# cxjyxxme/deep-online-video-stabilization

Measured on AMD Instinct MI355X. Metric: stabilized frames/sec (720p, before_ch=31), higher is better.
Workload: dtype f32 (bf16x3 split MFMA, f32 accumulate); 1 GPU; BASELINE.json configs[1]: v2_93 net, 1280x720, 1 stream(s)/GPU, batch=1 per stream, 13-ch stack from a 32-deep ring (lags 1,2,4,8,16,32; --before-ch 31 ignored as in the reference), ResNet-v2-50 regressor + 4x4 multi-grid warp + feedback; one independent stream set per GPU (replicas only); height=720, width=1280, streams_per_gpu=1, refine=1, operand_mode=4, launches_per_frame=64, hip_graph=True

## Files before the change

deep-online-video-stabilization_amd/csrc/conv.h:

```cpp
#pragma once
#include "common.h"

struct ConvArgs {
    const float* x;
    const float* w;
    float* y;
    const float* bias;
    const float* in_scale;
    const float* in_shift;
    const float* residual;
    const float* out_scale;
    const float* out_shift;
    const float* out_floor;
    float* partial;
    int N, H, W, Cin, Ho, Wo, Cout, KH, KW, stride, pad;
    int up;
    int res_H, res_W, res_stride;
    int relu_out;
    int x_ld, res_ld;
    int M, K;
    int splitk, steps_per_split;
    int cin_real;
    unsigned div_hw_mul, div_hw_shift, div_w_mul, div_w_shift;
    int rowrun;
    int in_scale_expected;
    int xcd_swizzle;
};

size_t conv_plan(ConvArgs& a);
struct Prof;
int conv_launch(const ConvArgs& a, hipStream_t st, Prof* prof = nullptr, int bf16_operands = 0, const float* w_img = nullptr,
                bool lowk_ring = false);

enum ConvFamily {
    CONV_IGEMM,
    CONV_RING,
    CONV_RING_KG,
    CONV_RING_PRO,
    CONV_PACKED,
    CONV_PACKED_KG2
};
struct ConvRoute {
    int family;
    int tile, bk, nbuf;
    int mode;
    int operand;
    int kg, pro;
    int reduce;
    int prof_kind;
};
ConvRoute conv_route(const ConvArgs& a, int operand_mode, bool has_image, bool bound, bool lowk_ring = false );
const char* conv_prof_kind_name(int kind);
size_t conv_weight_image_floats(int Cout, int K);
int launch_weight_split_image(const float* w, int Cout, int K, float* img, hipStream_t st);
struct WeightImageTable { long w_off[64], img_off[64], tprefix[65]; int Cout[64], K[64]; int n; };
void weight_image_table_add(WeightImageTable& t, long w_off, long img_off, int Cout, int K);
int launch_weight_split_images(const float* w_base, float* img_base, const WeightImageTable& t, hipStream_t st);
int conv_reduce_launches(const ConvArgs& a, int operand_mode = 0);

struct ConvPair { int m_tower, x_tower_floats ; long dx, dy, dres, dscale; };
bool conv_pair_supported(const ConvArgs& a);
int conv_launch_pair(const ConvArgs& a, const ConvPair& pr, hipStream_t st, Prof* prof = nullptr,
                     const float* w_img = nullptr );

bool conv_b2b_supported(const ConvArgs& c2, const ConvArgs& c3);
int conv_b2b_launch(const ConvArgs& c2, const ConvArgs& c3, hipStream_t st, Prof* prof = nullptr);

static inline void sn_fastdiv_make(unsigned d, unsigned& mul, unsigned& shift) {
    unsigned l = 0;
    while ((1ull << l) < d) ++l;
    mul = (unsigned)((((1ull << l) - d) << 32) / d + 1);
    shift = l;
}
#ifdef __HIPCC__
__device__ __forceinline__ int sn_fastdiv(int n, unsigned mul, unsigned shift) {
    return (int)((__umulhi(mul, (unsigned)n) + (unsigned)n) >> shift);
}
#endif
```

deep-online-video-stabilization_amd/csrc/conv.hip:

```cpp
#include "conv.h"
#include "prof.h"
#include <climits>
#include <cstdio>
#include <cstdlib>
#include <algorithm>
#include <string>
#include <vector>

#include "conv_kernel.h"
#include "conv_ring_kernel.h"
#include "conv_b2b_kernel.h"

template <int PAIR>
__device__ __forceinline__ void conv_splitk_reduce_body(const ConvArgs& p, const ConvPair& pr) {
    const size_t q = (size_t)blockIdx.x * 256 + threadIdx.x;
    const int c4n = p.Cout / 4;
    if (q >= (size_t)p.M * c4n) return;
    const int m = (int)(q / c4n);
    const int n = (int)(q - (size_t)m * c4n) * 4;
    const bool t1 = PAIR && m >= pr.m_tower;
    const size_t slab = (size_t)p.M * p.Cout;
    const float* src = p.partial + (size_t)m * p.Cout + n;
    float4 s = *reinterpret_cast<const float4*>(src);
    for (int z = 1; z < p.splitk; ++z) {
        const float4 t = *reinterpret_cast<const float4*>(src + z * slab);
        s.x += t.x; s.y += t.y; s.z += t.z; s.w += t.w;
    }
    if (p.bias != nullptr) {
        const float4 b = *reinterpret_cast<const float4*>(p.bias + n);
        s.x += b.x; s.y += b.y; s.z += b.z; s.w += b.w;
    }
    if (p.residual != nullptr) {
        size_t ri;
        if (p.res_stride == 1 && p.res_H == p.Ho && p.res_W == p.Wo) {
            ri = (size_t)m * p.res_ld + n;
        } else {
            const int img = sn_fastdiv(m, p.div_hw_mul, p.div_hw_shift);
            const int rr = m - img * (p.Ho * p.Wo);
            const int oy = sn_fastdiv(rr, p.div_w_mul, p.div_w_shift), ox = rr - oy * p.Wo;
            ri = (((size_t)img * p.res_H + oy * p.res_stride) * p.res_W + ox * p.res_stride) * p.res_ld + n;
        }
        const float4 t = *reinterpret_cast<const float4*>(p.residual + (t1 ? pr.dres : 0) + ri);
        s.x += t.x; s.y += t.y; s.z += t.z; s.w += t.w;
    }
    if (p.out_scale != nullptr) {
        const float4 a = *reinterpret_cast<const float4*>(p.out_scale + n), b = *reinterpret_cast<const float4*>(p.out_shift + n);
        s.x = __builtin_fmaf(s.x, a.x, b.x); s.y = __builtin_fmaf(s.y, a.y, b.y);
        s.z = __builtin_fmaf(s.z, a.z, b.z); s.w = __builtin_fmaf(s.w, a.w, b.w);
    }
    if (p.out_scale != nullptr && p.out_floor != nullptr) {
        const float4 f = *reinterpret_cast<const float4*>(p.out_floor + n);
        s.x = fmaxf(s.x, f.x); s.y = fmaxf(s.y, f.y); s.z = fmaxf(s.z, f.z); s.w = fmaxf(s.w, f.w);
    } else if (p.relu_out) {
        s.x = fmaxf(s.x, 0.f); s.y = fmaxf(s.y, 0.f); s.z = fmaxf(s.z, 0.f); s.w = fmaxf(s.w, 0.f);
    }
    *reinterpret_cast<float4*>(p.y + (t1 ? pr.dy : 0) + (size_t)m * p.Cout + n) = s;
}
__global__ __launch_bounds__(256) void conv_splitk_reduce_kernel(const ConvArgs p) {
    conv_splitk_reduce_body<0>(p, ConvPair{});
}
__global__ __launch_bounds__(256) void conv_splitk_reduce_pair_kernel(const ConvArgs p, const ConvPair pr) {
    conv_splitk_reduce_body<1>(p, pr);
}

enum TileId { T128x128 = 0, T128x64 = 1, T64x64 = 2 };

static void tile_dims(int t, int& bm, int& bn) {
    bm = (t == T64x64) ? 64 : 128;
    bn = (t == T128x128) ? 128 : 64;
}

static int env_int(const char* name, int dflt) {
    const char* v = getenv(name);
    return v ? atoi(v) : dflt;
}

struct ConvSwitches {
    int tile = env_int("STABNET_CONV_TILE", -1), splitk = env_int("STABNET_CONV_SPLITK", -1);
    int bk16 = env_int("STABNET_CONV_BK16", 0);
    int nbuf = env_int("STABNET_CONV_NBUF", 0);
    int tuning_table = env_int("STABNET_CONV_TUNING_TABLE", 1);
    int split_below = env_int("STABNET_CONV_SPLIT_BELOW", 400), split_target = env_int("STABNET_CONV_SPLIT_TARGET", 448);
    int xcd = env_int("STABNET_CONV_XCD", 1);
    int ring = env_int("STABNET_CONV_RING", 1), ring_wgs_per_cu = env_int("STABNET_CONV_RING_WGS_PER_CU", 3);
    int lowk_igemm = env_int("STABNET_CONV_LOWK_IGEMM", 1);
    int ring_pro = env_int("STABNET_CONV_RING_PRO", 1);
    int kgroups = env_int("STABNET_CONV_KGROUPS", 1), kgroups_pro = env_int("STABNET_CONV_KGROUPS_PRO", 1);
    int packed_kg2 = env_int("STABNET_CONV_PACKED_KG2", 1), packed_kg3 = env_int("STABNET_CONV_PACKED_KG3", 1);
    int packed_pro = env_int("STABNET_CONV_PACKED_PRO", 1);
    int packed_wgs_per_cu = env_int("STABNET_CONV_PACKED_WGS_PER_CU", 2);
    int b2b = env_int("STABNET_CONV_B2B", 1), b2b_wgs_per_cu = env_int("STABNET_CONV_B2B_WGS_PER_CU", 2);
};
static const ConvSwitches& sw() {
    static const ConvSwitches s;
    return s;
}

static int g_force_tile = -2, g_force_split = -1;
static int force_tile() { return g_force_tile == -2 ? sw().tile : g_force_tile; }
static int force_split() { return g_force_tile == -2 ? sw().splitk : g_force_split; }

static int conv_bk(const ConvArgs& a) { return (a.rowrun || (a.Cin % 32 == 0 && !sw().bk16)) ? 32 : 16; }
static int conv_total_steps(const ConvArgs& a) {
    if (a.rowrun) return a.KH * cdiv(a.KW * a.Cin, 32);
    return a.KH * a.KW * (a.Cin / conv_bk(a));
}

struct TuneEntry { int M, Cout, K, KH, ring, splitk; };
#include "conv_tuning_table.h"
#include "conv_tuning_table_packed.h"
static int g_tuning_profile = 0;
static std::vector<TuneEntry> g_tuning_runtime;

static int tuning_lookup(int M, int Cout, int K, int KH, int ring) {
    for (const TuneEntry& e : g_tuning_runtime)
        if (e.M == M && e.Cout == Cout && e.K == K && e.KH == KH && e.ring == ring) return e.splitk;
    if (sw().tuning_table && g_tuning_profile == 1)
        for (const TuneEntry& e : g_tuning_packed)
            if (e.M == M && e.Cout == Cout && e.K == K && e.KH == KH && e.ring == ring) return e.splitk;
    if (sw().tuning_table)
        for (const TuneEntry& e : g_tuning_builtin)
            if (e.M == M && e.Cout == Cout && e.K == K && e.KH == KH && e.ring == ring) return e.splitk;
    return 0;
}

static int pick_tile(const ConvArgs& a, int& splitk) {
    if (force_tile() >= 0) {
        const int steps0 = conv_total_steps(a);
        splitk = force_split() > 0 ? std::min(force_split(), steps0) : 1;
        return force_tile();
    }
    const int total_steps = conv_total_steps(a);
    const long blocks = (long)cdiv(a.M, 64) * cdiv(a.Cout, 64);
    const bool ring_path = a.rowrun || (a.in_scale_expected == 0 && a.up == 1 && a.Cin % 32 == 0);
    int s = tuning_lookup(a.M, a.Cout, a.K, a.KH, ring_path ? 1 : 0);
    const int thr = sw().split_below, target = sw().split_target;
    if (s > 0) {
        s = std::min(s, std::max(1, total_steps / 2));
    } else if (blocks < thr && a.Cout % 4 == 0) {
        s = (int)((target + blocks / 2) / blocks);
        s = std::min(s, std::max(1, total_steps / 8));
        s = std::min(s, 32);
    } else {
// ... 9 lines not shown
    a.K = a.rowrun ? a.KH * 32 * cdiv(a.KW * a.Cin, 32) : a.KH * a.KW * a.Cin;
    if (a.x_ld == 0) a.x_ld = a.Cin;
    if (a.res_ld == 0) a.res_ld = a.Cout;
    sn_fastdiv_make((unsigned)(a.Ho * a.Wo), a.div_hw_mul, a.div_hw_shift);
    sn_fastdiv_make((unsigned)a.Wo, a.div_w_mul, a.div_w_shift);
    int splitk = 1;
    (void)pick_tile(a, splitk);
    const int total_steps = conv_total_steps(a);
    a.steps_per_split = cdiv(total_steps, splitk);
    a.splitk = cdiv(total_steps, a.steps_per_split);
    return a.splitk > 1 ? (size_t)a.splitk * a.M * a.Cout * sizeof(float) : 0;
}

static void igemm_variant(const ConvArgs& a, int bm, int bn, int bk, int mode, int operand, int& nbuf_out, int& bf16_out) {
    const int nbuf = sw().nbuf;
    bf16_out = (bm == 64 && bn == 64 && bk == 32) ? operand : 0;
    const bool one_stage = nbuf == 1 || (nbuf == 0 && mode == 0 && bm == 64 && bn == 64 && a.M >= 32768);
    nbuf_out = (bf16_out != 1 && one_stage) ? 1 : 2;
}

static bool ring_eligible(const ConvArgs& a, int tile, bool has_prologue, bool lowk_ring = false) {
    if (a.rowrun) return true;
    if (!lowk_ring && sw().lowk_igemm && a.KH == 1 && a.KW == 1 && a.Cin == 64 && a.x_ld == a.Cin && a.out_floor == nullptr) return false;
    return sw().ring && tile == T64x64 && !has_prologue && a.up == 1 && a.Cin % 32 == 0 && !sw().bk16;
}

static bool ring_pro_vectors_ok(const ConvArgs& a) {
    if (a.in_scale == nullptr || a.in_shift == nullptr) return true;
    const long d = (long)(a.in_shift - a.in_scale);
    return d >= 0 && d < (1L << 30);
}
static bool ring_pro_geometry(const ConvArgs& a, int operand, bool has_prologue) {
    return sw().ring_pro && sw().ring && operand != 1 && !sw().bk16 && has_prologue && a.KH == 1 && a.KW == 1 && a.stride == 1 && a.pad == 0 &&
           a.up == 1 && a.Cin % 32 == 0 && !a.rowrun && a.x_ld == a.Cin;
}
static bool ring_pro_eligible(const ConvArgs& a, int operand) {
    return ring_pro_geometry(a, operand, a.in_scale != nullptr) && a.out_scale == nullptr && a.out_floor == nullptr && ring_pro_vectors_ok(a);
}

static int conv_kgroups(const ConvArgs& a, int operand, bool ring, bool has_prologue) {
    if (!sw().kgroups || a.splitk < 2 || operand == 1) return 1;
    if (a.steps_per_split * a.splitk != conv_total_steps(a)) return 1;
    if (ring && a.splitk == 3 && !a.rowrun) return 3;
    if (sw().kgroups_pro && !ring && a.splitk == 2 && ring_pro_geometry(a, operand, has_prologue) && ring_pro_vectors_ok(a)) return 2;
    return 1;
}

static int route_prof_kind(const ConvRoute& r) {
    switch (r.family) {
        case CONV_IGEMM:
            return PK_KERNEL_CONV_BASE + r.mode * 6 + r.tile * 2 + (r.bk == 32 ? 1 : 0) + (r.nbuf == 1 ? 18 : 0) + 36 * r.operand;
        case CONV_PACKED: return PK_KERNEL_CONV_PACKED + (r.pro ? 3 : r.mode);
        case CONV_PACKED_KG2: return PK_KERNEL_CONV_PACKED + (r.pro ? 6 : 4 + r.mode);
        default: break;
    }
    const int split = r.operand >= 2 ? PK_KERNEL_CONV_SPLIT + 8 * (r.operand - 2) : 0;
    if (r.family == CONV_RING) return split ? split + r.mode : PK_KERNEL_CONV_RING + r.mode + (r.operand ? 3 : 0);
    if (r.family == CONV_RING_PRO) return split ? split + 5 : PK_KERNEL_CONV_KG + 2;
    if (r.kg == 2) return split ? split + 6 : PK_KERNEL_CONV_KG + 3;
    return split ? split + 3 + r.mode : PK_KERNEL_CONV_KG + r.mode;
}

ConvRoute conv_route(const ConvArgs& a, int operand_mode, bool has_image, bool bound, bool lowk_ring) {
    const ConvSwitches& s = sw();
    const bool image = operand_mode == 4 && has_image;
    const int op = operand_mode == 4 ? 0 : operand_mode;
    int splitk_unused = 1;
    const int t = pick_tile(a, splitk_unused);
    const bool t64 = t == T64x64, bk32 = conv_bk(a) == 32;
    const bool has_pro = bound ? a.in_scale != nullptr : a.in_scale_expected != 0;
    const bool ring = ring_eligible(a, t, has_pro, lowk_ring && image);
    const bool slabs = !bound || a.splitk == 1 || a.partial != nullptr;
    int kg = t64 ? conv_kgroups(a, op, ring, has_pro) : 1;
    if (image && s.packed_kg3 && ring && kg == 3 && a.K % 32 == 0 && slabs) kg = 1;
    const bool pro = kg == 1 && !ring && t64 && bk32 && (bound ? ring_pro_eligible(a, op) : ring_pro_geometry(a, op, has_pro));
    const bool packed_pro = image && s.packed_pro && !ring && t64 && bk32 && ring_pro_geometry(a, op, has_pro) &&
                            (!bound || a.out_floor == nullptr)  && ring_pro_vectors_ok(a) && slabs;
    if (packed_pro) kg = 1;
    const bool packed = (image && ring && kg == 1 && a.K % 32 == 0) || packed_pro;
    const bool packed_kg2 = packed && s.packed_kg2 && a.splitk == 2 && !a.rowrun && a.steps_per_split * 2 == conv_total_steps(a);
    if (packed_kg2) kg = 2;

    ConvRoute r{};
    r.tile = t;
    r.bk = bk32 ? 32 : 16;
    r.mode = (a.up > 1 || a.rowrun) ? 2 : (a.pad == 0 ? 0 : 1);
    r.operand = op;
    r.kg = kg;
    r.reduce = (a.splitk > 1 && kg == 1) ? 1 : 0;
    if (packed) {
        r.family = packed_kg2 ? CONV_PACKED_KG2 : CONV_PACKED;
        r.operand = 4;
        r.pro = packed_pro ? 1 : 0;
    } else if (pro) {
        r.family = CONV_RING_PRO;
        r.pro = 1;
    } else if (kg > 1) {
        r.family = CONV_RING_KG;
        r.pro = kg == 2 ? 1 : 0;
    } else if (ring) {
        r.family = CONV_RING;
    } else {
        int bm, bn;
        tile_dims(t, bm, bn);
        r.family = CONV_IGEMM;
        igemm_variant(a, bm, bn, r.bk, r.mode, op, r.nbuf, r.operand);
    }
    r.prof_kind = route_prof_kind(r);
    return r;
}

int conv_reduce_launches(const ConvArgs& a, int operand_mode) {
    return a.splitk < 2 ? 0 : conv_route(a, operand_mode, operand_mode == 4, false).reduce;
}

const char* conv_prof_kind_name(int kind) {
    static const std::vector<std::string> names = [] {
        std::vector<std::string> v(PK_KERNEL_CONV_BASE + 144);
        char buf[96];
        auto ring = [&](int family, int mode, int operand, int kg, int pro) {
            ConvRoute r{};
            r.family = family; r.mode = mode; r.operand = operand; r.kg = kg; r.pro = pro;
            snprintf(buf, sizeof(buf), "conv_ring_f32_kernel<%d, %d, %d, %d>", mode, operand, kg, pro);
            v[route_prof_kind(r)] = buf;
        };
        for (int operand = 0; operand < 4; ++operand) {
            for (int mode = 0; mode < 3; ++mode) ring(CONV_RING, mode, operand, 1, 0);
            if (operand == 1) continue;
            ring(CONV_RING_KG, 0, operand, 3, 0); ring(CONV_RING_KG, 1, operand, 3, 0);
            ring(CONV_RING_PRO, 0, operand, 1, 1); ring(CONV_RING_KG, 0, operand, 2, 1);
        }
        for (int mode = 0; mode < 3; ++mode) ring(CONV_PACKED, mode, 4, 1, 0);
        ring(CONV_PACKED, 0, 4, 1, 1);
        ring(CONV_PACKED_KG2, 0, 4, 2, 0); ring(CONV_PACKED_KG2, 1, 4, 2, 0); ring(CONV_PACKED_KG2, 0, 4, 2, 1);
        for (int i = 0; i < 144; ++i) {
            ConvRoute r{};
            r.family = CONV_IGEMM;
            r.operand = i / 36; r.nbuf = 2 - i / 18 % 2; r.mode = i / 6 % 3; r.tile = i / 2 % 3; r.bk = (i & 1) ? 32 : 16;
            int bm, bn;
            tile_dims(r.tile, bm, bn);
            snprintf(buf, sizeof(buf), "conv_igemm_f32_kernel<%d, %d, %d, %d, %d, %d, %d, %d>", bm, bn, r.bk, bm / 2, bn / 2, r.mode, r.nbuf, r.operand);
            v[route_prof_kind(r)] = buf;
        }
        for (int i = 0; i < 4; ++i) {
            snprintf(buf, sizeof(buf), "conv_igemm_f32_pair_kernel<64, 64, %d, 32, 32, %d>", (i & 1) ? 32 : 16, i / 2);
            v[PK_KERNEL_CONV_PAIR + i] = buf;
        }
        v[PK_KERNEL_CONV_B2B] = "conv_b2b_f32_kernel<2>";
        v[PK_KERNEL_CONV_B2B + 1] = "conv_b2b_f32_kernel<4>";
        return v;
    }();
    return (kind >= 0 && kind < (int)names.size() && !names[kind].empty()) ? names[kind].c_str() : nullptr;
}

template <int BM, int BN, int BK, int WM, int WN, int MODE, int NBUF, int BF16 = 0>
static int launch_one_nb(const ConvArgs& a, hipStream_t st) {
    constexpr size_t lds_op = NBUF * (size_t)(BM + BN) * (BK + 4) * sizeof(float);
    constexpr size_t lds_epi = 4 * (size_t)SN_EPI_WAVE_BYTES;
    constexpr size_t lds = lds_op > lds_epi ? lds_op : lds_epi;
    static bool configured = false;
    auto kern = conv_igemm_f32_kernel<BM, BN, BK, WM, WN, MODE, NBUF, BF16>;
    if (!configured) {
        if (lds > 64 * 1024) {
            hipError_t e = hipFuncSetAttribute(reinterpret_cast<const void*>(kern),
                                               hipFuncAttributeMaxDynamicSharedMemorySize, (int)lds);
            if (e != hipSuccess) {
                stabnet_set_error("conv: hipFuncSetAttribute(%zu B LDS) failed: %s", lds, hipGetErrorString(e));
                return STABNET_ERR_LAUNCH;
            }
        }
        configured = true;
    }
    dim3 grid(cdiv(a.M, BM), cdiv(a.Cout, BN), a.splitk);
    kern<<<grid, 256, lds, st>>>(a);
    SN_LAUNCH_CHECK("conv_igemm_f32_kernel");
    return STABNET_OK;
}

template <int BM, int BN, int BK, int WM, int WN, int MODE>
static int launch_one_t(const ConvRoute& r, const ConvArgs& a, hipStream_t st) {
    if constexpr (BM == 64 && BN == 64 && BK == 32) {
        if (r.operand == 1) return launch_one_nb<BM, BN, BK, WM, WN, MODE, 2, 1>(a, st);
        else if (r.operand == 2) return r.nbuf == 1 ? launch_one_nb<BM, BN, BK, WM, WN, MODE, 1, 2>(a, st) : launch_one_nb<BM, BN, BK, WM, WN, MODE, 2, 2>(a, st);
        else if (r.operand == 3) return r.nbuf == 1 ? launch_one_nb<BM, BN, BK, WM, WN, MODE, 1, 3>(a, st) : launch_one_nb<BM, BN, BK, WM, WN, MODE, 2, 3>(a, st);
    }
    return r.nbuf == 1 ? launch_one_nb<BM, BN, BK, WM, WN, MODE, 1>(a, st) : launch_one_nb<BM, BN, BK, WM, WN, MODE, 2>(a, st);
}
// ... 20 lines not shown
    static int cached = 0;
    if (cached == 0) {
        int dev = 0, n = 0;
        if (hipGetDevice(&dev) != hipSuccess || hipDeviceGetAttribute(&n, hipDeviceAttributeMultiprocessorCount, dev) != hipSuccess || n <= 0) {
            stabnet_set_error("conv: cannot read the CU count");
            return STABNET_ERR_LAUNCH;
        }
        cached = n;
    }
    cus = cached;
    return STABNET_OK;
}
static int g_reserved_cus = 0;
static int usable_cus(int cus) { return std::max(cus / 8, cus - std::max(0, g_reserved_cus)); }

template <int B>
static bool launch_ring_operand(const ConvRoute& r, const ConvArgs& a, int grid, hipStream_t st) {
    const int key = 100 * r.mode + 10 * r.kg + r.pro;
    if (key == 10) { conv_ring_f32_kernel<0, B><<<grid, 256, 0, st>>>(a); return true; }
    if (key == 110) { conv_ring_f32_kernel<1, B><<<grid, 256, 0, st>>>(a); return true; }
    if (key == 210) { conv_ring_f32_kernel<2, B><<<grid, 256, 0, st>>>(a); return true; }
    if constexpr (B != 1) {
        if (key == 11) { conv_ring_f32_kernel<0, B, 1, 1><<<grid, 256, 0, st>>>(a); return true; }
        if (key == 21) { conv_ring_f32_kernel<0, B, 2, 1><<<grid, 512, 0, st>>>(a); return true; }
    }
    if constexpr (B == 0 || B == 2 || B == 3) {
        if (key == 30) { conv_ring_f32_kernel<0, B, 3><<<grid, 768, 0, st>>>(a); return true; }
        if (key == 130) { conv_ring_f32_kernel<1, B, 3><<<grid, 768, 0, st>>>(a); return true; }
    }
    if constexpr (B == 4) {
        if (key == 20) { conv_ring_f32_kernel<0, B, 2, 0><<<grid, 512, 0, st>>>(a); return true; }
        if (key == 120) { conv_ring_f32_kernel<1, B, 2, 0><<<grid, 512, 0, st>>>(a); return true; }
    }
    return false;
}

static int launch_ring_route(const ConvRoute& r, const ConvArgs& a, hipStream_t st) {
    int cus = 0;
    if (const int rc = device_cus(cus)) return rc;
    const int per_cu = r.kg > 1 ? 1 : (r.operand == 4 ? sw().packed_wgs_per_cu : sw().ring_wgs_per_cu);
    const long ntiles = (long)cdiv(a.M, 64) * cdiv(a.Cout, 64) * (r.kg > 1 ? 1 : a.splitk);
    const int grid = (int)std::min<long>(ntiles, (long)per_cu * usable_cus(cus));
    bool ok = false;
    switch (r.operand) {
        case 0: ok = launch_ring_operand<0>(r, a, grid, st); break;
        case 1: ok = launch_ring_operand<1>(r, a, grid, st); break;
        case 2: ok = launch_ring_operand<2>(r, a, grid, st); break;
        case 3: ok = launch_ring_operand<3>(r, a, grid, st); break;
        case 4: ok = launch_ring_operand<4>(r, a, grid, st); break;
        default: break;
    }
    SN_REQUIRE(ok, "conv: no conv_ring_f32_kernel<%d, %d, %d, %d>", r.mode, r.operand, r.kg, r.pro);
    SN_LAUNCH_CHECK("conv_ring_f32_kernel");
    return STABNET_OK;
}

size_t conv_weight_image_floats(int Cout, int K) { return (size_t)cdiv(Cout, 64) * (size_t)(K / 32) * 3072; }

__device__ __forceinline__ unsigned weight_split_head(float& x0, float& x1) {
    const float top = __builtin_bit_cast(float, 0x7F7F0000u), fmax = __builtin_bit_cast(float, 0x7F7FFFFFu);
    const float h0 = (fabsf(x0) > top && fabsf(x0) <= fmax) ? copysignf(top, x0) : x0;
    const float h1 = (fabsf(x1) > top && fabsf(x1) <= fmax) ? copysignf(top, x1) : x1;
    const unsigned p = sn_pack_bf16(h0, h1);
    x0 = sn_sub_f32(x0, __builtin_bit_cast(float, p << 16));
    x1 = sn_sub_f32(x1, __builtin_bit_cast(float, p & 0xffff0000u));
    return p;
}
__device__ __forceinline__ SnSplit3 weight_split3(const f32x4 x) {
    float a = x.x, b = x.y, c = x.z, d = x.w;
    typedef unsigned u32x2 __attribute__((ext_vector_type(2)));
    u32x2 h, m, l;
    h.x = weight_split_head(a, b); h.y = weight_split_head(c, d);
    m.x = sn_split_level(a, b); m.y = sn_split_level(c, d);
    l.x = sn_pack_bf16(a, b); l.y = sn_pack_bf16(c, d);
    SnSplit3 s;
    s.h = __builtin_bit_cast(sn_bf16x4, h); s.m = __builtin_bit_cast(sn_bf16x4, m); s.l = __builtin_bit_cast(sn_bf16x4, l);
    return s;
}

__device__ __forceinline__ void weight_split_image_thread(const float* __restrict__ w, int Cout, int K, uint4* __restrict__ img, long i) {
    const int steps = K / 32;
    const int lane = (int)(i & 63), j = (int)((i >> 6) & 1), wn = (int)((i >> 7) & 1);
    const long ts = i >> 8;
    const int ks = (int)(ts % steps), nt = (int)(ts / steps);
    const int n = nt * 64 + wn * 32 + (lane & 31), g = lane >> 5;
    f32x4 lo = {0.f, 0.f, 0.f, 0.f}, hi = lo;
    if (n < Cout) {
        const float* r = w + (size_t)n * K + ks * 32 + 16 * j + 4 * g;
        lo = *reinterpret_cast<const f32x4*>(r);
        hi = *reinterpret_cast<const f32x4*>(r + 8);
    }
    const SnSplit3 a = weight_split3(lo), b = weight_split3(hi);
    uint4* out = img + ts * 768 + (size_t)(wn * 6 + j) * 64 + lane;
    out[0] = __builtin_bit_cast(uint4, SN_CAT8(a.h, b.h));
    out[2 * 64] = __builtin_bit_cast(uint4, SN_CAT8(a.m, b.m));
    out[4 * 64] = __builtin_bit_cast(uint4, SN_CAT8(a.l, b.l));
}

__global__ __launch_bounds__(256) void weight_split_image_kernel(const float* __restrict__ w, int Cout, int K, uint4* __restrict__ img) {
    const long i = (long)blockIdx.x * 256 + threadIdx.x;
    if (i >= (long)((Cout + 63) / 64) * (K / 32) * 256) return;
    weight_split_image_thread(w, Cout, K, img, i);
}

__global__ __launch_bounds__(256) void weight_split_images_kernel(const float* __restrict__ w_base, float* __restrict__ img_base, const WeightImageTable t) {
    const long i = (long)blockIdx.x * 256 + threadIdx.x;
    if (i >= t.tprefix[t.n]) return;
    int e = 0;
    while (i >= t.tprefix[e + 1]) ++e;
    weight_split_image_thread(w_base + t.w_off[e], t.Cout[e], t.K[e], reinterpret_cast<uint4*>(img_base + t.img_off[e]), i - t.tprefix[e]);
}

void weight_image_table_add(WeightImageTable& t, long w_off, long img_off, int Cout, int K) {
    if (t.n == 0) t.tprefix[0] = 0;
    t.w_off[t.n] = w_off; t.img_off[t.n] = img_off; t.Cout[t.n] = Cout; t.K[t.n] = K;
    t.tprefix[t.n + 1] = t.tprefix[t.n] + (long)cdiv(Cout, 64) * (K / 32) * 256;
    ++t.n;
}

int launch_weight_split_images(const float* w_base, float* img_base, const WeightImageTable& t, hipStream_t st) {
    if (t.n == 0) return STABNET_OK;
    SN_REQUIRE(w_base && img_base && t.n <= 64, "weight images: bad table");
    weight_split_images_kernel<<<(unsigned)(t.tprefix[t.n] >> 8), 256, 0, st>>>(w_base, img_base, t);
    SN_LAUNCH_CHECK("weight_split_images_kernel");
    return STABNET_OK;
}

int launch_weight_split_image(const float* w, int Cout, int K, float* img, hipStream_t st) {
    SN_REQUIRE(w && img && Cout > 0 && K > 0 && K % 32 == 0, "weight image: K=%d must be a multiple of 32", K);
    const long total = (long)cdiv(Cout, 64) * (K / 32) * 256;
    weight_split_image_kernel<<<cdiv(total, 256), 256, 0, st>>>(w, Cout, K, reinterpret_cast<uint4*>(img));
    SN_LAUNCH_CHECK("weight_split_image_kernel");
    return STABNET_OK;
}

int conv_launch(const ConvArgs& a, hipStream_t st, Prof* prof, int bf16_operands, const float* w_img, bool lowk_ring) {
    SN_REQUIRE(a.rowrun || a.Cin % 16 == 0, "conv: Cin=%d must be a multiple of 16 (pad the channels)", a.Cin);
    SN_REQUIRE(!a.rowrun || (a.in_scale == nullptr && a.up == 1 && a.KH <= 8 && cdiv(a.KW * a.Cin, 32) <= 4),
               "conv: row-run operand needs no prologue, KH <= 8 and KW*Cin <= 128");
    SN_REQUIRE(a.Cout % 4 == 0, "conv: Cout=%d must be a multiple of 4", a.Cout);
    SN_REQUIRE(a.splitk >= 1 && a.steps_per_split >= 1 && a.div_hw_mul != 0, "conv: conv_plan() not called");
    SN_REQUIRE(a.splitk == 1 || a.partial != nullptr, "conv: split-K needs a workspace");
    const ConvRoute r = conv_route(a, bf16_operands, w_img != nullptr, true, lowk_ring);
    SN_REQUIRE(r.family != CONV_IGEMM || a.x_ld == a.Cin, "conv: a strided input (x_ld %d != Cin %d) needs the ring kernel", a.x_ld, a.Cin);
    const bool rec = prof != nullptr && prof->begin(st);
    int rc;
    switch (r.family) {
        case CONV_IGEMM: rc = launch_igemm(r, a, st); break;
        case CONV_PACKED:
        case CONV_PACKED_KG2: {
            ConvArgs b = a;
            b.w = w_img;
            rc = launch_ring_route(r, b, st);
            break;
        }
        default: rc = launch_ring_route(r, a, st); break;
    }
    if (rec) prof->end(st, r.prof_kind, 2.0 * a.M * (double)(a.KH * a.KW * (a.cin_real ? a.cin_real : a.Cin)) * a.Cout,
                       4.0 * ((double)a.N * a.H * a.W * a.Cin + (double)a.K * a.Cout + (double)a.M * a.Cout * (r.reduce ? a.splitk : 1) +
                              ((a.residual != nullptr && !r.reduce) ? (double)a.M * a.Cout : 0.0)),
                       a.M, a.Cout, a.K, a.splitk);
    if (rc) return rc;
    if (r.reduce) {
        const size_t q = (size_t)a.M * (a.Cout / 4);
        const bool rec2 = prof != nullptr && prof->begin(st);
        conv_splitk_reduce_kernel<<<cdiv((long)q, 256), 256, 0, st>>>(a);
        if (rec2) prof->end(st, PK_KERNEL_SPLITK_REDUCE, 0.0, 4.0 * (double)a.M * a.Cout * (a.splitk + 1 + (a.residual != nullptr ? 1 : 0)));
        SN_LAUNCH_CHECK("conv_splitk_reduce_kernel");
    }
    return STABNET_OK;
}

bool conv_pair_supported(const ConvArgs& a) {
    int splitk_unused = 1;
    const int t = pick_tile(a, splitk_unused);
    const bool pro = a.in_scale != nullptr || a.in_scale_expected;
    return t == T64x64 && !ring_eligible(a, t, pro) && a.up == 1 && !a.rowrun && (a.x_ld == 0 || a.x_ld == a.Cin);
}

template <int BK, int MODE>
static int launch_pair_one(const ConvArgs& a, const ConvPair& pr, hipStream_t st) {
    constexpr size_t lds = 2 * (size_t)(64 + 64) * (BK + 4) * sizeof(float);
    static_assert(lds >= 4 * (size_t)SN_EPI_WAVE_BYTES && lds <= 64 * 1024, "LDS of the 64x64 tile");
    dim3 grid(cdiv(a.M, 64), cdiv(a.Cout, 64), a.splitk);
    conv_igemm_f32_pair_kernel<64, 64, BK, 32, 32, MODE><<<grid, 256, lds, st>>>(a, pr);
    SN_LAUNCH_CHECK("conv_igemm_f32_pair_kernel");
    return STABNET_OK;
}

int conv_launch_pair(const ConvArgs& a, const ConvPair& pr, hipStream_t st, Prof* prof, const float* w_img) {
    SN_REQUIRE(a.Cin % 16 == 0 && a.Cout % 4 == 0, "conv pair: Cin %% 16 and Cout %% 4 must be 0");
    SN_REQUIRE(a.splitk >= 1 && a.steps_per_split >= 1 && a.div_hw_mul != 0, "conv pair: conv_plan() not called");
    SN_REQUIRE(a.splitk == 1 || a.partial != nullptr, "conv pair: split-K needs a workspace");
    SN_REQUIRE(conv_pair_supported(a), "conv pair: the plan of this shape is not the 64x64 register-staged launch");
    SN_REQUIRE(pr.m_tower > 0 && pr.m_tower % 64 == 0 && a.M == 2 * pr.m_tower, "conv pair: tower rows %d must be a multiple of 64 (M %d)",
               pr.m_tower, a.M);
    const bool bk32 = conv_bk(a) == 32;
    const int mode = a.pad == 0 ? 0 : 1;
    const bool pro = bk32 && ring_pro_eligible(a, 0) && pr.dx == pr.dscale - (long)pr.m_tower * a.Cin && pr.dy == pr.dscale - (long)pr.m_tower * a.Cout &&
                     (a.residual == nullptr || pr.dres == pr.dscale - (long)(a.N / 2) * a.res_H * a.res_W * a.res_ld);
    const bool packed = pro && w_img != nullptr && a.K % 32 == 0 && a.splitk == 1;
    ConvRoute r{};
    r.family = packed ? CONV_PACKED : CONV_RING_PRO;
    r.operand = packed ? 4 : 0;
    r.kg = r.pro = 1;
    const bool rec = prof != nullptr && prof->begin(st);
// ... 119 lines not shown
        return 0;
    ConvArgs b = a;
    b.in_scale_expected = 1;
    return std::max(conv_plan(a), conv_plan(b));
}

int stabnet_conv2d_fwd_ex(const float* x, const float* w_ohwi, const float* bias, const float* in_scale,
                          const float* in_shift, const float* residual, int res_H, int res_W, int res_stride,
                          const float* out_scale, const float* out_shift, float* y, int N, int H, int W, int Cin,
                          int Cout, int KH, int KW, int stride, int pad, int relu_out, void* workspace,
                          size_t workspace_bytes, void* stream);

int stabnet_conv2d_fwd(const float* x, const float* w_ohwi, const float* bias, const float* in_scale,
                       const float* in_shift, const float* residual, int res_H, int res_W, int res_stride, float* y,
                       int N, int H, int W, int Cin, int Cout, int KH, int KW, int stride, int pad, int relu_out,
                       void* workspace, size_t workspace_bytes, void* stream) {
    return stabnet_conv2d_fwd_ex(x, w_ohwi, bias, in_scale, in_shift, residual, res_H, res_W, res_stride, nullptr, nullptr,
                                 y, N, H, W, Cin, Cout, KH, KW, stride, pad, relu_out, workspace, workspace_bytes, stream);
}

int stabnet_conv2d_fwd_ex(const float* x, const float* w_ohwi, const float* bias, const float* in_scale,
                          const float* in_shift, const float* residual, int res_H, int res_W, int res_stride,
                          const float* out_scale, const float* out_shift, float* y, int N, int H, int W, int Cin,
                          int Cout, int KH, int KW, int stride, int pad, int relu_out, void* workspace,
                          size_t workspace_bytes, void* stream) {
    SN_REQUIRE(x && w_ohwi && y, "conv2d_fwd: null pointer");
    SN_REQUIRE((out_scale == nullptr) == (out_shift == nullptr), "conv2d_fwd: out_scale and out_shift go together");
    ConvArgs a;
    int rc = fill_args(a, x, w_ohwi, bias, in_scale, in_shift, residual, res_H, res_W, res_stride, y, N, H, W, Cin, Cout,
                       KH, KW, stride, pad, relu_out);
    if (rc) return rc;
    const size_t need = conv_plan(a);
    if (need > workspace_bytes || (need > 0 && workspace == nullptr)) {
        stabnet_set_error("conv2d_fwd: workspace %zu B < %zu B needed", workspace_bytes, need);
        return STABNET_ERR_WORKSPACE;
    }
    a.partial = static_cast<float*>(workspace);
    a.out_scale = out_scale;
    a.out_shift = out_shift;
    return conv_launch(a, (hipStream_t)stream);
}

size_t stabnet_conv_weight_image_floats(int Cout, int KH, int KW, int Cin) {
    const int K = KH * KW * Cin;
    return (Cout > 0 && K > 0 && K % 32 == 0) ? conv_weight_image_floats(Cout, K) : 0;
}

int stabnet_conv_weight_split_image(const float* w_ohwi, int Cout, int KH, int KW, int Cin, float* w_img, void* stream) {
    SN_REQUIRE(w_ohwi && w_img, "conv_weight_split_image: null pointer");
    SN_REQUIRE(Cin % 32 == 0, "conv_weight_split_image: Cin=%d must be a multiple of 32", Cin);
    return launch_weight_split_image(w_ohwi, Cout, KH * KW * Cin, w_img, (hipStream_t)stream);
}

int stabnet_conv2d_fwd_packed(const float* x, const float* w_ohwi, const float* w_img, const float* bias, const float* in_scale,
                              const float* in_shift, const float* residual, int res_H, int res_W, int res_stride,
                              const float* out_scale, const float* out_shift, float* y, int N, int H, int W, int Cin,
                              int Cout, int KH, int KW, int stride, int pad, int relu_out, int splitk, void* workspace,
                              size_t workspace_bytes, void* stream) {
    SN_REQUIRE(x && w_ohwi && w_img && y, "conv2d_fwd_packed: null pointer");
    SN_REQUIRE((out_scale == nullptr) == (out_shift == nullptr), "conv2d_fwd_packed: out_scale and out_shift go together");
    ConvArgs a;
    int rc = fill_args(a, x, w_ohwi, bias, in_scale, in_shift, residual, res_H, res_W, res_stride, y, N, H, W, Cin, Cout,
                       KH, KW, stride, pad, relu_out);
    if (rc) return rc;
    size_t need = conv_plan(a);
    if (splitk > 0) {
        const int total = conv_total_steps(a);
        a.steps_per_split = cdiv(total, std::min(splitk, total));
        a.splitk = cdiv(total, a.steps_per_split);
        need = a.splitk > 1 ? (size_t)a.splitk * a.M * a.Cout * sizeof(float) : 0;
    }
    if (need > workspace_bytes || (need > 0 && workspace == nullptr)) {
        stabnet_set_error("conv2d_fwd_packed: workspace %zu B < %zu B needed", workspace_bytes, need);
        return STABNET_ERR_WORKSPACE;
    }
    a.partial = static_cast<float*>(workspace);
    a.out_scale = out_scale;
    a.out_shift = out_shift;
    return conv_launch(a, (hipStream_t)stream, nullptr, 4, w_img);
}

int stabnet_conv3x3_conv1x1_fwd(const float* x, int x_ld, const float* w2_ohwi, const float* mid_scale, const float* mid_shift,
                                const float* w3_ohwi, const float* bias3, const float* residual, int res_H, int res_W,
                                int res_stride, int res_ld, const float* out_scale, const float* out_shift, float* y, int N, int H,
                                int W, int C, int Cout, int stride, int relu_out, void* stream) {
    SN_REQUIRE(x && w2_ohwi && mid_scale && mid_shift && w3_ohwi && y, "conv3x3_conv1x1_fwd: null pointer");
    SN_REQUIRE((out_scale == nullptr) == (out_shift == nullptr), "conv3x3_conv1x1_fwd: out_scale and out_shift go together");
    ConvArgs c2, c3;
    int rc = fill_args(c2, x, w2_ohwi, nullptr, nullptr, nullptr, nullptr, 0, 0, 1, nullptr, N, H, W, C, C, 3, 3, stride, 1, 1);
    if (rc) return rc;
    c2.x_ld = x_ld;
    (void)conv_plan(c2);
    c2.out_scale = mid_scale;
    c2.out_shift = mid_shift;
    rc = fill_args(c3, nullptr, w3_ohwi, bias3, nullptr, nullptr, residual, res_H, res_W, res_stride, y, N, c2.Ho, c2.Wo, C, Cout,
                   1, 1, 1, 0, relu_out);
    if (rc) return rc;
    c3.res_ld = res_ld;
    (void)conv_plan(c3);
    c3.out_scale = out_scale;
    c3.out_shift = out_shift;
    SN_REQUIRE(conv_b2b_supported(c2, c3), "conv3x3_conv1x1_fwd: C must be 64 or 128, Cout a multiple of C, stride 1 or 2");
    return conv_b2b_launch(c2, c3, (hipStream_t)stream);
}

}
```

deep-online-video-stabilization_amd/csrc/prof.h:

```cpp
#pragma once
#include <vector>
#include "common.h"

enum {
    PK_KERNEL_PAD = 1, PK_KERNEL_POOL = 2, PK_KERNEL_GAP = 3, PK_KERNEL_FC = 4, PK_KERNEL_MESH = 5,
    PK_KERNEL_WARP = 6, PK_KERNEL_ASSEMBLE = 7, PK_KERNEL_PUSH = 8, PK_KERNEL_SPLITK_REDUCE = 9, PK_KERNEL_WGRAD = 10, PK_KERNEL_HEAD = 20,
    PK_KERNEL_MJPEG_TRANSFORM = 30, PK_KERNEL_MJPEG_ENTROPY = 31, PK_KERNEL_MJPEG_LAYOUT = 32, PK_KERNEL_MJPEG_GATHER = 33 ,
    PK_KERNEL_INGEST_GREY_ROWS = 34, PK_KERNEL_INGEST_GREY_COLS = 35, PK_KERNEL_INGEST_COLOUR = 36 ,
    PK_KERNEL_MAP_SHRINK = 37, PK_KERNEL_REMAP_SRC = 38, PK_KERNEL_REMAP_SRC4 = 39 ,
    PK_KERNEL_REMAP_WIN = 60, PK_KERNEL_REMAP_WIN4 = 61 ,
    PK_KERNEL_REMAP_WIN_DEV = 62, PK_KERNEL_REMAP_WIN4_DEV = 63 ,
    PK_KERNEL_WGRAD_SAME = 11 ,
    PK_KERNEL_CONV_PAIR = 80 , PK_KERNEL_CONV_KG = 84 , PK_KERNEL_CONV_RING = 90 ,
    PK_KERNEL_CONV_PACKED = 70 ,
    PK_KERNEL_CONV_B2B = 96 ,
    PK_KERNEL_CONV_SPLIT = 40 ,
    PK_KERNEL_CONV_BASE = 100
};

struct Prof {
    std::vector<hipEvent_t> ev;
    std::vector<int> kind;
    std::vector<double> flops, bytes;
    std::vector<int> shape;
    int cap = 0, n = 0;
    bool begin(hipStream_t st) {
        if (n >= cap) return false;
        (void)hipEventRecord(ev[2 * n], st);
        return true;
    }
    void end(hipStream_t st, int k, double f, double b, int sm = 0, int sn = 0, int sk = 0, int ss = 0) {
        (void)hipEventRecord(ev[2 * n + 1], st);
        kind[n] = k; flops[n] = f; bytes[n] = b;
        shape[4 * n] = sm; shape[4 * n + 1] = sn; shape[4 * n + 2] = sk; shape[4 * n + 3] = ss;
        ++n;
    }
};
```

include/stabnet_hip.h:

```cpp
#ifndef STABNET_HIP_H
#define STABNET_HIP_H

#include <stddef.h>
#include <stdint.h>

#ifdef __cplusplus
extern "C" {
#endif

const char* stabnet_last_error(void);
int stabnet_abi_version(void);


int stabnet_get_4_pts(const float* theta, int N, int grid_h, int grid_w, float do_crop_rate,
                      float* pts1, float* pts2, float* Hs, void* stream);

int stabnet_transformer_fwd(const float* pts2, const float* U, int N, int H, int W, int C, int grid_h, int grid_w,
                            float* out, float* black, float* x_map, float* y_map, float* Hs, void* stream);

int stabnet_warp_fwd(const float* theta, const float* U, int N, int H, int W, int C, int grid_h, int grid_w,
                     float do_crop_rate, float* out, float* black, float* x_map, float* y_map, float* Hs,
                     float* pts2, void* stream);

int stabnet_maps_from_hs_fwd(const float* Hs, const float* U, int N, int H, int W, int C, int grid_h, int grid_w,
                             float* out, float* black, float* x_map, float* y_map, void* stream);

int stabnet_interp_fwd(const float* im, const float* x, const float* y, int N, int H, int W, int C, float* out,
                       void* stream);


size_t stabnet_conv2d_workspace_bytes(int N, int H, int W, int Cin, int Cout, int KH, int KW, int stride, int pad);
void stabnet_conv_tuning_override(int tile, int splitk);
void stabnet_conv_tuning_table_set(int M, int Cout, int K, int KH, int ring, int splitk);
void stabnet_conv_tuning_profile(int profile);
int stabnet_conv2d_fwd(const float* x, const float* w_ohwi, const float* bias, const float* in_scale,
                       const float* in_shift, const float* residual, int res_H, int res_W, int res_stride, float* y,
                       int N, int H, int W, int Cin, int Cout, int KH, int KW, int stride, int pad, int relu_out,
                       void* workspace, size_t workspace_bytes, void* stream);
int stabnet_conv2d_fwd_ex(const float* x, const float* w_ohwi, const float* bias, const float* in_scale,
                          const float* in_shift, const float* residual, int res_H, int res_W, int res_stride,
                          const float* out_scale, const float* out_shift, float* y, int N, int H, int W, int Cin,
                          int Cout, int KH, int KW, int stride, int pad, int relu_out, void* workspace,
                          size_t workspace_bytes, void* stream);
size_t stabnet_conv_weight_image_floats(int Cout, int KH, int KW, int Cin);
int stabnet_conv_weight_split_image(const float* w_ohwi, int Cout, int KH, int KW, int Cin, float* w_img, void* stream);
int stabnet_conv2d_fwd_packed(const float* x, const float* w_ohwi, const float* w_img, const float* bias, const float* in_scale,
                              const float* in_shift, const float* residual, int res_H, int res_W, int res_stride,
                              const float* out_scale, const float* out_shift, float* y, int N, int H, int W, int Cin,
                              int Cout, int KH, int KW, int stride, int pad, int relu_out, int splitk, void* workspace,
                              size_t workspace_bytes, void* stream);
int stabnet_conv3x3_conv1x1_fwd(const float* x, int x_ld, const float* w2_ohwi, const float* mid_scale, const float* mid_shift,
                                const float* w3_ohwi, const float* bias3, const float* residual, int res_H, int res_W,
                                int res_stride, int res_ld, const float* out_scale, const float* out_shift, float* y, int N, int H,
                                int W, int C, int Cout, int stride, int relu_out, void* stream);

int stabnet_net_create(void** net, int N, int H, int W, int in_ch, int n_theta, int keep_activations);
void stabnet_net_destroy(void* net);
int stabnet_net_set_bf16_operands(void* net, int on);
int stabnet_net_num_params(const void* net);
int stabnet_net_param_info(const void* net, int idx, char* name, int name_cap, long* offset, int* kind, int* dims4,
                           int* aux);
size_t stabnet_net_param_floats(const void* net);
size_t stabnet_net_trainable_floats(const void* net);
size_t stabnet_net_bn_channels(const void* net);
size_t stabnet_net_workspace_bytes(const void* net);
double stabnet_net_flops(const void* net);
int stabnet_net_num_launches(const void* net);
int stabnet_deploy_frame_launches(const void* net, int grid_h, int grid_w);
int stabnet_net_activation_info(const void* net, const char* name, long* offset, int* dims4);

int stabnet_net_fold_bn(const void* net, const float* params, float* fold, float eps, void* stream);
size_t stabnet_net_fold_floats(const void* net);

int stabnet_backbone_fwd_infer(const void* net, const float* params, const float* fold, const float* x_tensor,
                               float* theta, void* workspace, size_t workspace_bytes, void* stream, void* prof);


int stabnet_pad_channels(const float* x, float* y, long npix, int C, int Cp, void* stream);

int stabnet_stem_repack(const float* w, float* out, int Cout, int KH, int KW, int CinPad, int Cin, void* stream);

int stabnet_merge_vectors(const float* b_sc, const float* scale1, const float* shift1, int depth, int dbn, float* out, void* stream);

int stabnet_bn_fold(const float* gamma, const float* beta, const float* mean, const float* var, float eps, int G, float* scale,
                    float* shift, void* stream);

int stabnet_max_pool_fwd(const float* x, float* y, int N, int H, int W, int C, int Ho, int Wo, int k, int stride, int pt, int pl,
                         const float* scale, const float* shift, void* stream);

size_t stabnet_gap_partial_floats(int N, int HW, int C);
int stabnet_gap_bn_relu(const float* x, const float* scale, const float* shift, int N, int HW, int C, float* out, float* partial,
                        size_t partial_floats, void* stream);

int stabnet_fc_fwd(const float* x, const float* w, const float* b, float* y, int M, int K, int Nout, int relu, void* stream);

int stabnet_head_fused_supported(int N, int C, const int* fc_dims);
size_t stabnet_head_gap_partial_floats(int N, int HW, int C);
int stabnet_head_gap_fc1(const float* x, const float* scale, const float* shift, int N, int HW, int C, float* partial,
                         size_t partial_floats, float* gap_out, const float* w, const float* b, float* y, int Nout, void* stream);
int stabnet_head_theta_mesh(const float* x, const float* w, const float* b, int N, int K, int n_theta, float* theta, int grid_h,
                            int grid_w, float do_crop_rate, float* Hs, int* head_adv, int depth, const float* prefetch_src, int pf_H,
                            int pf_W, void* stream);

// ... 207 lines not shown
```

Before: 710.3 frames/s.

## Add A-stationary packed kernel for large-M 1x1 convs with small K

Adds a new conv family for 1x1 stride-1 convolutions with K<=256 and Cout>=256. Each block splits its 32-row activation tile into bf16 hi/mid/lo planes once and keeps them in LDS, then streams the packed weight image through triple-buffered registers across several Cout blocks. This avoids re-splitting and reloading activations for every Cout tile. The cost is fewer, longer blocks and reduced occupancy because of the 48KB LDS, and the routing thresholds on M were picked by hand. A query entry point for the route kind is also added.

```diff
diff --git a/deep-online-video-stabilization_amd/csrc/conv.h b/deep-online-video-stabilization_amd/csrc/conv.h
--- a/deep-online-video-stabilization_amd/csrc/conv.h
+++ b/deep-online-video-stabilization_amd/csrc/conv.h
@@ -38,7 +38,8 @@
     CONV_RING_KG,
     CONV_RING_PRO,
     CONV_PACKED,
-    CONV_PACKED_KG2
+    CONV_PACKED_KG2,
+    CONV_ASTAT
 };
 struct ConvRoute {
     int family;
@@ -48,6 +49,7 @@
     int kg, pro;
     int reduce;
     int prof_kind;
+    int astat_bm;
 };
 ConvRoute conv_route(const ConvArgs& a, int operand_mode, bool has_image, bool bound, bool lowk_ring = false );
 const char* conv_prof_kind_name(int kind);
diff --git a/deep-online-video-stabilization_amd/csrc/conv.hip b/deep-online-video-stabilization_amd/csrc/conv.hip
--- a/deep-online-video-stabilization_amd/csrc/conv.hip
+++ b/deep-online-video-stabilization_amd/csrc/conv.hip
@@ -9,6 +9,7 @@
 
 #include "conv_kernel.h"
 #include "conv_ring_kernel.h"
+#include "conv_astat_kernel.h"
 #include "conv_b2b_kernel.h"
 
 template <int PAIR>
@@ -89,6 +90,8 @@
     int packed_kg2 = env_int("STABNET_CONV_PACKED_KG2", 1), packed_kg3 = env_int("STABNET_CONV_PACKED_KG3", 1);
     int packed_pro = env_int("STABNET_CONV_PACKED_PRO", 1);
     int packed_wgs_per_cu = env_int("STABNET_CONV_PACKED_WGS_PER_CU", 2);
+    int astat = env_int("STABNET_CONV_ASTAT", 1), astat_min_m = env_int("STABNET_CONV_ASTAT_MIN_M", 0);
+    int astat_min_cout = env_int("STABNET_CONV_ASTAT_MIN_COUT", 256);
     int b2b = env_int("STABNET_CONV_B2B", 1), b2b_wgs_per_cu = env_int("STABNET_CONV_B2B_WGS_PER_CU", 2);
 };
 static const ConvSwitches& sw() {
@@ -204,6 +207,7 @@
             return PK_KERNEL_CONV_BASE + r.mode * 6 + r.tile * 2 + (r.bk == 32 ? 1 : 0) + (r.nbuf == 1 ? 18 : 0) + 36 * r.operand;
         case CONV_PACKED: return PK_KERNEL_CONV_PACKED + (r.pro ? 3 : r.mode);
         case CONV_PACKED_KG2: return PK_KERNEL_CONV_PACKED + (r.pro ? 6 : 4 + r.mode);
+        case CONV_ASTAT: return PK_KERNEL_CONV_ASTAT;
         default: break;
     }
     const int split = r.operand >= 2 ? PK_KERNEL_CONV_SPLIT + 8 * (r.operand - 2) : 0;
@@ -232,6 +236,10 @@
     const bool packed = (image && ring && kg == 1 && a.K % 32 == 0) || packed_pro;
     const bool packed_kg2 = packed && s.packed_kg2 && a.splitk == 2 && !a.rowrun && a.steps_per_split * 2 == conv_total_steps(a);
     if (packed_kg2) kg = 2;
+    const int astat_min_m = s.astat_min_m > 0 ? s.astat_min_m : ((long)a.Cout * a.K >= 128 * 1024 ? 2048 : 8192);
+    const bool astat = packed && !packed_pro && !packed_kg2 && kg == 1 && a.splitk == 1 && s.astat && !lowk_ring && !a.rowrun &&
+                       a.KH == 1 && a.KW == 1 && a.stride == 1 && a.pad == 0 && a.up == 1 && a.K <= 256 && a.Cout >= s.astat_min_cout &&
+                       a.M >= astat_min_m;
 
     ConvRoute r{};
     r.tile = t;
@@ -240,7 +248,11 @@
     r.operand = op;
     r.kg = kg;
     r.reduce = (a.splitk > 1 && kg == 1) ? 1 : 0;
-    if (packed) {
+    if (astat) {
+        r.family = CONV_ASTAT;
+        r.operand = 4;
+        r.astat_bm = 32;
+    } else if (packed) {
         r.family = packed_kg2 ? CONV_PACKED_KG2 : CONV_PACKED;
         r.operand = 4;
         r.pro = packed_pro ? 1 : 0;
@@ -285,6 +297,12 @@
         for (int mode = 0; mode < 3; ++mode) ring(CONV_PACKED, mode, 4, 1, 0);
         ring(CONV_PACKED, 0, 4, 1, 1);
         ring(CONV_PACKED_KG2, 0, 4, 2, 0); ring(CONV_PACKED_KG2, 1, 4, 2, 0); ring(CONV_PACKED_KG2, 0, 4, 2, 1);
+        {
+            ConvRoute r{};
+            r.family = CONV_ASTAT; r.astat_bm = 32;
+            snprintf(buf, sizeof(buf), "conv_astat_f32_kernel<%d>", r.astat_bm);
+            v[route_prof_kind(r)] = buf;
+        }
         for (int i = 0; i < 144; ++i) {
             ConvRoute r{};
             r.family = CONV_IGEMM;
@@ -411,6 +429,21 @@
     }
     SN_REQUIRE(ok, "conv: no conv_ring_f32_kernel<%d, %d, %d, %d>", r.mode, r.operand, r.kg, r.pro);
     SN_LAUNCH_CHECK("conv_ring_f32_kernel");
+    return STABNET_OK;
+}
+
+static int launch_astat(const ConvRoute& r, const ConvArgs& a, hipStream_t st) {
+    int cus = 0;
+    if (const int rc = device_cus(cus)) return rc;
+    const int bm = r.astat_bm;
+    SN_REQUIRE(bm == 32 && a.K % 32 == 0 && (size_t)bm * a.K * 6 <= (size_t)SN_ASTAT_A_BYTES && a.splitk == 1,
+               "conv: the A-stationary kernel takes BM %d x K %d without a K split only if the planes fit %d bytes", bm, a.K, SN_ASTAT_A_BYTES);
+    const int mtiles = cdiv(a.M, bm), nblk = 2 * cdiv(a.Cout, 64);
+    int groups = (int)std::min<long>(cdiv(nblk, 4), std::max<long>(1, 2L * usable_cus(cus) / mtiles));
+    groups = cdiv(nblk, 4 * cdiv(cdiv(nblk, groups), 4));
+    const dim3 grid(mtiles, groups);
+    conv_astat_f32_kernel<32><<<grid, 256, 0, st>>>(a);
+    SN_LAUNCH_CHECK("conv_astat_f32_kernel");
     return STABNET_OK;
 }
 
@@ -511,6 +544,12 @@
             ConvArgs b = a;
             b.w = w_img;
             rc = launch_ring_route(r, b, st);
+            break;
+        }
+        case CONV_ASTAT: {
+            ConvArgs b = a;
+            b.w = w_img;
+            rc = launch_astat(r, b, st);
             break;
         }
         default: rc = launch_ring_route(r, a, st); break;
@@ -736,6 +775,26 @@
     return launch_weight_split_image(w_ohwi, Cout, KH * KW * Cin, w_img, (hipStream_t)stream);
 }
 
+static size_t plan_packed(ConvArgs& a, int splitk) {
+    size_t need = conv_plan(a);
+    if (splitk > 0) {
+        const int total = conv_total_steps(a);
+        a.steps_per_split = cdiv(total, std::min(splitk, total));
+        a.splitk = cdiv(total, a.steps_per_split);
+        need = a.splitk > 1 ? (size_t)a.splitk * a.M * a.Cout * sizeof(float) : 0;
+    }
+    return need;
+}
+
+int stabnet_conv2d_packed_kind(int N, int H, int W, int Cin, int Cout, int KH, int KW, int stride, int pad, int prologue, int splitk) {
+    ConvArgs a;
+    if (fill_args(a, nullptr, nullptr, nullptr, nullptr, nullptr, nullptr, 0, 0, 1, nullptr, N, H, W, Cin, Cout, KH, KW, stride, pad, 0))
+        return STABNET_ERR_BAD_ARG;
+    a.in_scale_expected = prologue ? 1 : 0;
+    (void)plan_packed(a, splitk);
+    return conv_route(a, 4, true, false).prof_kind;
+}
+
 int stabnet_conv2d_fwd_packed(const float* x, const float* w_ohwi, const float* w_img, const float* bias, const float* in_scale,
                               const float* in_shift, const float* residual, int res_H, int res_W, int res_stride,
                               const float* out_scale, const float* out_shift, float* y, int N, int H, int W, int Cin,
@@ -747,13 +806,7 @@
     int rc = fill_args(a, x, w_ohwi, bias, in_scale, in_shift, residual, res_H, res_W, res_stride, y, N, H, W, Cin, Cout,
                        KH, KW, stride, pad, relu_out);
     if (rc) return rc;
-    size_t need = conv_plan(a);
-    if (splitk > 0) {
-        const int total = conv_total_steps(a);
-        a.steps_per_split = cdiv(total, std::min(splitk, total));
-        a.splitk = cdiv(total, a.steps_per_split);
-        need = a.splitk > 1 ? (size_t)a.splitk * a.M * a.Cout * sizeof(float) : 0;
-    }
+    const size_t need = plan_packed(a, splitk);
     if (need > workspace_bytes || (need > 0 && workspace == nullptr)) {
         stabnet_set_error("conv2d_fwd_packed: workspace %zu B < %zu B needed", workspace_bytes, need);
         return STABNET_ERR_WORKSPACE;
diff --git a/deep-online-video-stabilization_amd/csrc/conv_astat_kernel.h b/deep-online-video-stabilization_amd/csrc/conv_astat_kernel.h
--- /dev/null
+++ b/deep-online-video-stabilization_amd/csrc/conv_astat_kernel.h
@@ -0,0 +1,105 @@
+#pragma once
+#include "conv_kernel.h"
+
+constexpr int SN_ASTAT_A_BYTES = 48 * 1024;
+
+template <int BM>
+__global__ __launch_bounds__(256, 2) void conv_astat_f32_kernel(const ConvArgs p) {
+    static_assert(BM == 32 || BM == 64, "one or two 32-row blocks");
+    constexpr int RB = BM / 32;
+    typedef unsigned u32x2 __attribute__((ext_vector_type(2)));
+    __shared__ __attribute__((aligned(16))) unsigned char lds[SN_ASTAT_A_BYTES + 4 * SN_EPI_WAVE_BYTES];
+
+    const int tid = threadIdx.x, lane = tid & 63, wave = __builtin_amdgcn_readfirstlane(tid >> 6);
+    const int steps = p.K >> 5, kq = 2 * steps;
+    const ConvTile tile = conv_tile_of_block(p);
+    const int m0 = tile.mt * BM, grp = tile.nt;
+
+    {
+        const int r = tid >> 3, sub = tid & 7;
+        const unsigned ent = (unsigned)((r + 32 * (sub & 1)) * 16 + 8 * ((sub >> 1) & 1));
+#pragma unroll
+        for (int rb = 0; rb < RB; ++rb) {
+            const int row = min(m0 + rb * 32 + r, p.M - 1);
+            const float* src = p.x + (size_t)row * p.x_ld + sub * 4;
+            for (int ks0 = 0; ks0 < steps; ks0 += 4) {
+                f32x4 v[4];
+#pragma unroll
+                for (int i = 0; i < 4; ++i) v[i] = *reinterpret_cast<const f32x4*>(src + 32 * min(ks0 + i, steps - 1));
+                __builtin_amdgcn_sched_barrier(0);
+#pragma unroll
+                for (int i = 0; i < 4; ++i) {
+                    float a = v[i].x, b = v[i].y, c = v[i].z, d = v[i].w;
+                    u32x2 h, m, l;
+                    h.x = sn_split_level(a, b); h.y = sn_split_level(c, d);
+                    m.x = sn_split_level(a, b); m.y = sn_split_level(c, d);
+                    l.x = sn_pack_bf16(a, b); l.y = sn_pack_bf16(c, d);
+                    unsigned char* dst = lds + (unsigned)((rb * kq + 2 * min(ks0 + i, steps - 1) + (sub >> 2)) * 3072) + ent;
+                    *reinterpret_cast<u32x2*>(dst) = h;
+                    *reinterpret_cast<u32x2*>(dst + 1024) = m;
+                    *reinterpret_cast<u32x2*>(dst + 2048) = l;
+                }
+            }
+        }
+    }
+    __syncthreads();
+
+    const int nblk = 2 * ((p.Cout + 63) >> 6);
+    const int bpg = (((nblk + (int)gridDim.y - 1) / (int)gridDim.y) + 3) & ~3;
+    const int b_end = min(min(nblk, (grp + 1) * bpg), (p.Cout + 31) >> 5);
+    int b = grp * bpg + wave;
+    if (b >= b_end) return;
+    const unsigned scratch = (unsigned)(size_t)(__attribute__((address_space(3))) void*)lds + (unsigned)(SN_ASTAT_A_BYTES + wave * SN_EPI_WAVE_BYTES);
+    const f32x4* lp = reinterpret_cast<const f32x4*>(p.w) + ((size_t)(b >> 1) * steps * 12 + (b & 1) * 6) * 64 + lane;
+    const unsigned char* afrag = lds + lane * 16;
+    const int items = ((b_end - b + 3) >> 2) * steps;
+    int l_item = 0, l_ks = 0;
+    auto load = [&](f32x4 (&dst)[6]) {
+#pragma unroll
+        for (int i = 0; i < 6; ++i) dst[i] = lp[i * 64];
+        const int adv = l_item + 1 >= items ? 0 : (l_ks + 1 < steps ? 768 : 768 * (steps + 1));
+        lp += adv;
+        ++l_item;
+        l_ks = l_ks + 1 < steps ? l_ks + 1 : 0;
+        __builtin_amdgcn_sched_barrier(0);
+    };
+    f32x16 acc[RB][1];
+    auto zero = [&]() {
+#pragma unroll
+        for (int rb = 0; rb < RB; ++rb)
+#pragma unroll
+            for (int e = 0; e < 16; ++e) acc[rb][0][e] = 0.f;
+    };
+    int ks = 0;
+    auto item = [&](const f32x4 (&B)[6]) {
+#pragma unroll
+        for (int j = 0; j < 2; ++j) {
+#pragma unroll
+            for (int rb = 0; rb < RB; ++rb) {
+                const unsigned char* ap = afrag + (unsigned)((rb * kq + 2 * ks + j) * 3072);
+                SnPlanes A;
+                A.h = *reinterpret_cast<const sn_u32x4*>(ap);
+                A.m = *reinterpret_cast<const sn_u32x4*>(ap + 1024);
+                A.l = *reinterpret_cast<const sn_u32x4*>(ap + 2048);
+                sn_mfma_split3_pk(acc[rb][0], A, B[j], B[2 + j], B[4 + j]);
+            }
+        }
+        if (++ks == steps) {
+            conv_epilogue<RB, 1>(acc, p, m0, b * 32, lane, 0, scratch);
+            b += 4;
+            ks = 0;
+            zero();
+        }
+    };
+    f32x4 B0[6], B1[6], B2[6];
+    zero();
+    load(B0);
+    load(B1);
+    for (int it = 0; it < items; it += 3) {
+        load(B2); item(B0);
+        if (it + 1 >= items) break;
+        load(B0); item(B1);
+        if (it + 2 >= items) break;
+        load(B1); item(B2);
+    }
+}
diff --git a/deep-online-video-stabilization_amd/csrc/prof.h b/deep-online-video-stabilization_amd/csrc/prof.h
--- a/deep-online-video-stabilization_amd/csrc/prof.h
+++ b/deep-online-video-stabilization_amd/csrc/prof.h
@@ -13,6 +13,7 @@
     PK_KERNEL_WGRAD_SAME = 11 ,
     PK_KERNEL_CONV_PAIR = 80 , PK_KERNEL_CONV_KG = 84 , PK_KERNEL_CONV_RING = 90 ,
     PK_KERNEL_CONV_PACKED = 70 ,
+    PK_KERNEL_CONV_ASTAT = 77 ,
     PK_KERNEL_CONV_B2B = 96 ,
     PK_KERNEL_CONV_SPLIT = 40 ,
     PK_KERNEL_CONV_BASE = 100
diff --git a/include/stabnet_hip.h b/include/stabnet_hip.h
--- a/include/stabnet_hip.h
+++ b/include/stabnet_hip.h
@@ -49,6 +49,7 @@
                               const float* out_scale, const float* out_shift, float* y, int N, int H, int W, int Cin,
                               int Cout, int KH, int KW, int stride, int pad, int relu_out, int splitk, void* workspace,
                               size_t workspace_bytes, void* stream);
+int stabnet_conv2d_packed_kind(int N, int H, int W, int Cin, int Cout, int KH, int KW, int stride, int pad, int prologue, int splitk);
 int stabnet_conv3x3_conv1x1_fwd(const float* x, int x_ld, const float* w2_ohwi, const float* mid_scale, const float* mid_shift,
                                 const float* w3_ohwi, const float* bias3, const float* residual, int res_H, int res_W,
                                 int res_stride, int res_ld, const float* out_scale, const float* out_shift, float* y, int N, int H,
```

Result: faster. 728.4 frames/s, median of 6 (+2.6%).
